# Jennifer03333333332/Soft-Rendering-Toolsets

Hardware: AMD Instinct MI355X
Metric: Mrays/s (higher is better)
Workload: dtype f32; 1 GPU; Scotty3D Pathtracer: Cornell box (cbox: area light + MIS, mirror + glass spheres), 1024x1024, 64 spp per step (52 steps = 3328 spp; 32 steps = BASELINE configs[3] 2048 spp), depth 8, BVH on; tiles=32x32 round-robin over ranks, collective=none (1 GPU), seed=0

## Files before the change

include/srt_pt_debug.h:

```cpp
#ifndef SRT_PT_DEBUG_H
#define SRT_PT_DEBUG_H

#include "srt_pt.h"

#ifdef __cplusplus
extern "C" {
#endif

int srt_pt_set_kernel(srt_pt* pt, int mode);
int srt_pt_section_cycles(srt_pt* pt, uint64_t out[8], int reset);

int srt_pt_kernel_time(srt_pt* pt, int enable, double* total_ms, uint64_t* launches);

int srt_pt_stream_times(srt_pt* pt, int enable, double ms_out[4], uint64_t* generations);
int srt_pt_stream_counters(srt_pt* pt, uint64_t out[4], int reset);
int srt_pt_kernel_form(srt_pt* pt, int* form);

int srt_pt_counters(srt_pt* pt, uint64_t out[8]);
int srt_pt_scene_counts(srt_pt* pt, uint64_t out[8]);
int srt_pt_refit_count(srt_pt* pt, uint64_t* refits);
int srt_pt_top_refit_count(srt_pt* pt, uint64_t* refits);
int srt_pt_top_refit_pending(srt_pt* pt, uint64_t out[2]);
int srt_pt_mesh_refit_pending(srt_pt* pt, uint64_t out[2]);
long srt_pt_dump_lights(srt_pt* pt, int from_device, uint32_t* heads, float* mats, size_t cap_lights, float* tris, size_t cap_tris);
int srt_pt_dump_shading(srt_pt* pt, int from_device, uint32_t counts[2], srt_pt_material* materials, size_t cap_materials, uint32_t* light_heads,
                        float* light_values, size_t cap_lights, uint32_t* env_type, float env_radiance[3]);
int srt_pt_math_cos_sin(srt_pt* pt, const float* x, size_t n, float* cos_out, float* sin_out);
int srt_pt_math_sincos2(srt_pt* pt, const float* x, size_t n, float* cos_out, float* sin_out);
int srt_pt_math_atan2(srt_pt* pt, const float* y, const float* x, size_t n, float* out);
int srt_pt_math_acos(srt_pt* pt, const float* x, size_t n, float* out);
int srt_pt_math_hypot(srt_pt* pt, const float* x, const float* y, size_t n, float* out);
int srt_pt_rig_posed_host(uint32_t njoints, const int32_t* parent, const float* extents, const float base[3], const float* rest_pose,
                          const uint32_t* knot_offsets, const float* knot_times, const float* knot_quats, float t, float* euler_out, float* posed_out);
int srt_pt_rig_step_ik_host(uint32_t njoints, const int32_t* parent, const float* extents, float* pose_inout, const uint32_t* handle_joints,
                            const float* targets, const uint8_t* enabled, uint32_t nhandles, uint32_t calls);
int srt_pt_emitter_advance_host(srt_pt_emitter* em, float dt, uint32_t* substeps, uint32_t* spawns_out, uint32_t cap, int* cleared, double schedule_out[2]);

int srt_pt_math_exp(srt_pt* pt, const float* x, size_t n, float* out);
int srt_pt_math_pow(srt_pt* pt, const float* x, const float* y, size_t n, float* out);
int srt_pt_math_div_sqrt(srt_pt* pt, const float* in, size_t lanes, int shared_c2, float* out);
int srt_pt_math_tri_verdict(srt_pt* pt, const float* in, size_t lanes, float* out);
int srt_pt_math_leaf_fold(srt_pt* pt, const float* in, size_t lanes, float* out);
int srt_pt_math_sphere_batch(srt_pt* pt, const float* in, size_t lanes, float* out);
int srt_pt_math_box_sweep(srt_pt* pt, const float* in, size_t lanes, float* out);
int srt_pt_math_point_affine(srt_pt* pt, const float* in, size_t lanes, float* out);

int srt_pt_live_resources(uint64_t out[3]);

#ifdef __cplusplus
}
#endif
#endif
```

soft-rendering-toolsets_amd/_pt_bindings.py:

```python
from __future__ import annotations

import ctypes
import os
import weakref
from ctypes import POINTER, c_float, c_int, c_long, c_size_t, c_uint32, c_uint64, c_void_p

import numpy as np


class PtMaterial(ctypes.Structure):
    _fields_ = [("type", c_uint32), ("a", c_float * 3), ("b", c_float * 3), ("ior", c_float)]


LOGGED_RAY_DTYPE = np.dtype([("point", np.float32, 3), ("dir", np.float32, 3), ("t", np.float32), ("pixel", np.uint32),
                             ("sample", np.uint32), ("bounce", np.uint32)])
SRT_CANCELLED = 1


class SrtCancelled(Exception):
    """A render call returned SRT_CANCELLED: srt_pt_cancel cut it short, its output was not written."""


_HIP_MEMCPY_D2H = 2

# ... 136 lines not shown
    lib.srt_pt_dump_bvh.restype = c_long
    lib.srt_pt_counters.argtypes = [c_void_p, c_void_p]
    lib.srt_pt_math_cos_sin.argtypes = [c_void_p, c_void_p, c_size_t, c_void_p, c_void_p]
    lib.srt_pt_math_sincos2.argtypes = [c_void_p, c_void_p, c_size_t, c_void_p, c_void_p]
    lib.srt_pt_math_acos.argtypes = [c_void_p, c_void_p, c_size_t, c_void_p]
    lib.srt_pt_math_atan2.argtypes = [c_void_p, c_void_p, c_void_p, c_size_t, c_void_p]
    lib.srt_pt_set_elision.argtypes = [c_void_p, c_int]
    lib.srt_pt_rays_elided.argtypes = [c_void_p, POINTER(c_uint64), c_int]
    lib.srt_pt_set_normal_colors.argtypes = [c_void_p, c_int]
    lib.srt_pt_group_set_normal_colors.argtypes = [c_void_p, c_int]
    lib.srt_pt_set_dynamic_lights.argtypes = [c_void_p, c_int]
    lib.srt_pt_group_set_dynamic_lights.argtypes = [c_void_p, c_int]
    lib.srt_pt_dump_lights.argtypes = [c_void_p, c_int, c_void_p, c_void_p, c_size_t, c_void_p, c_size_t]
    lib.srt_pt_dump_lights.restype = c_long
    lib.srt_pt_math_exp.argtypes = [c_void_p, c_void_p, c_size_t, c_void_p]
    lib.srt_pt_math_pow.argtypes = [c_void_p, c_void_p, c_void_p, c_size_t, c_void_p]
    lib.srt_pt_tonemap.argtypes = [c_void_p, c_void_p, c_uint32, c_uint32, c_float, c_void_p]
    lib.srt_pt_tonemap_device.argtypes = [c_void_p, c_void_p, c_void_p, c_uint32, c_uint32, c_float, c_void_p]
    lib.srt_pt_math_div_sqrt.argtypes = [c_void_p, c_void_p, c_size_t, ctypes.c_int, c_void_p]
    lib.srt_pt_math_tri_verdict.argtypes = [c_void_p, c_void_p, c_size_t, c_void_p]
    lib.srt_pt_math_leaf_fold.argtypes = [c_void_p, c_void_p, c_size_t, c_void_p]
    lib.srt_pt_math_box_sweep.argtypes = [c_void_p, c_void_p, c_size_t, c_void_p]
    lib.srt_pt_math_point_affine.argtypes = [c_void_p, c_void_p, c_size_t, c_void_p]
    lib.srt_pt_math_sphere_batch.argtypes = [c_void_p, c_void_p, c_size_t, c_void_p]
    lib.srt_pt_sync.argtypes = [c_void_p]
    lib.srt_pt_cancel.argtypes = [c_void_p]
    lib.srt_pt_cancel_requested.argtypes = [c_void_p]
    lib.srt_pt_clear_cancel.argtypes = [c_void_p]
    lib.srt_pt_set_ray_log.argtypes = [c_void_p, c_uint32]
    lib.srt_pt_read_ray_log.argtypes = [c_void_p, c_void_p, c_size_t, POINTER(c_size_t), POINTER(c_uint64)]
    lib.srt_pt_read_ray_log_stream.argtypes = [c_void_p, c_void_p, c_void_p, c_size_t, POINTER(c_size_t), POINTER(c_uint64)]
    lib.srt_pt_group_render_epoch_lane.argtypes = [c_void_p, c_int, c_uint64, c_uint32, c_uint32, POINTER(c_void_p), POINTER(c_void_p)]
    lib.srt_pt_group_cancel.argtypes = [c_void_p]
    lib.srt_pt_group_clear_cancel.argtypes = [c_void_p]
    lib.srt_pt_group_set_ray_log.argtypes = [c_void_p, c_uint32]
    lib.srt_pt_group_read_ray_log.argtypes = [c_void_p, c_int, c_void_p, c_size_t, POINTER(c_size_t), POINTER(c_uint64)]
    lib.srt_pt_max_samples_per_launch.argtypes = [c_void_p, POINTER(c_uint32)]
    lib.srt_pt_accumulator_floats.argtypes = [c_void_p, POINTER(c_size_t)]
    lib.srt_pt_render_samples_device.argtypes = [c_void_p, c_void_p, c_uint64, c_uint32, c_uint32]
    lib.srt_pt_fold_epochs_device.argtypes = [c_void_p, c_void_p, c_uint32, c_uint32, c_uint32, c_uint32, c_void_p]
    lib.srt_pt_accumulator_tiles_device.argtypes = [c_void_p, c_void_p, c_void_p, c_void_p]
    lib.srt_pt_group_reset_accumulator.argtypes = [c_void_p]
    lib.srt_pt_group_max_samples_per_launch.argtypes = [c_void_p, POINTER(c_uint32)]
    lib.srt_pt_group_render_samples.argtypes = [c_void_p, c_int, c_uint64, c_uint32, c_uint32]
    lib.srt_pt_group_wait_lane.argtypes = [c_void_p, c_int]
    lib.srt_pt_group_fold.argtypes = [c_void_p, c_int, c_uint32, c_uint32, c_uint32, c_uint32]
# ... 1158 lines not shown
        self._check(self._lib, self._lib.srt_pt_math_sphere_batch(self._ctx, _p(planes), n, _p(out)))
        form = lambda b: {"hit": out[b:b + 9:3].T != 0, "t": out[b + 1:b + 9:3].T.copy(), "dist": out[b + 2:b + 9:3].T.copy()}
        return form(0), form(9), out[18:21].T.copy(), out[21] != 0

    def math_box_sweep(self, box, org, inv, times):
        box, org, inv, times = _f32(box).reshape(-1, 6), _f32(org).reshape(-1, 3), _f32(inv).reshape(-1, 3), _f32(times).reshape(-1, 2)
        n = len(box)
        assert len(org) == n and len(inv) == n and len(times) == n and n > 0
        planes = np.ascontiguousarray(np.concatenate([box, org, inv, times], axis=1).T)
        out = np.zeros((6, n), np.float32)
        self._check(self._lib, self._lib.srt_pt_math_box_sweep(self._ctx, _p(planes), n, _p(out)))
        form = lambda b: {"hit": out[b] != 0, "tx": out[b + 1].copy(), "ty": out[b + 2].copy()}
        return form(0), form(3)

    def math_point_affine(self, mats, points):
        mats, points = _f32(mats).reshape(-1, 16), _f32(points).reshape(-1, 3)
        W, n = len(mats), len(points)
        assert n == 64 * W and W > 0
        buf = np.ascontiguousarray(np.concatenate([mats.ravel(), points.T.ravel()]), np.float32)
        out = np.zeros((7, n), np.float32)
        self._check(self._lib, self._lib.srt_pt_math_point_affine(self._ctx, _p(buf), n, _p(out)))
        return out[0:3].T.copy(), out[3:6].T.copy(), out[6].reshape(W, 64)[:, 0] != 0

    def math_cos_sin(self, x):
        x = _f32(x)
        c, s = np.zeros_like(x), np.zeros_like(x)
        self._check(self._lib, self._lib.srt_pt_math_cos_sin(self._ctx, _p(x), len(x), _p(c), _p(s)))
        return c, s

    def math_sincos2(self, x):
        x = _f32(x)
        c, s = np.zeros_like(x), np.zeros_like(x)
        self._check(self._lib, self._lib.srt_pt_math_sincos2(self._ctx, _p(x), len(x), _p(c), _p(s)))
        return c, s

    def sync(self) -> None:
        self._check(self._lib, self._lib.srt_pt_sync(self._ctx))


class PathtracerGroup:

    def __init__(self, devices):
        from . import SrtError, _check, load_library

        self._SrtError, self._check = SrtError, _check
        self._lib = load_library()
# ... 252 lines not shown
```

soft-rendering-toolsets_amd/csrc/pt_probe.hip:

```cpp
#include <hip/hip_runtime.h>

#include "pt_anim.h"
#include "pt_context.h"
#include "pt_device.h"
#include "srt_pt_debug.h"

#include "pt_trace.h"

namespace srt {

__global__ void pt_math_kernel(const float* __restrict__ x, size_t n, float* __restrict__ c, float* __restrict__ s) {
  const size_t i = (size_t)blockIdx.x * blockDim.x + threadIdx.x;
  if (i < n) { c[i] = srt_cosf(x[i]); s[i] = srt_sinf(x[i]); }
}

__global__ void pt_sincos2_kernel(const float* __restrict__ x, size_t n, float* __restrict__ c, float* __restrict__ s) {
  const size_t i = (size_t)blockIdx.x * blockDim.x + threadIdx.x;
  float cv, sv;
  srt_sincosf2(x[i < n ? i : n - 1], cv, sv);
  if (i < n) { c[i] = cv; s[i] = sv; }
}

__global__ void pt_acos_kernel(const float* __restrict__ x, size_t n, float* __restrict__ out) {
  const size_t i = (size_t)blockIdx.x * blockDim.x + threadIdx.x;
// ... 175 lines not shown
  const float bx[6] = {v[0], v[1], v[2], v[3], v[4], v[5]};
  const V3 org = v3(v[6], v[7], v[8]), inv = v3(v[9], v[10], v[11]);
  float ax = v[12], ay = v[13], bxx = v[12], bxy = v[13];
  const bool ha = box_hit_inv(bx, org, inv, ax, ay);
  const bool hb = box_hit_rec(bx, org, inv, bxx, bxy);
  out[i] = ha ? 1.0f : 0.0f; out[lanes + i] = ax; out[2 * lanes + i] = ay;
  out[3 * lanes + i] = hb ? 1.0f : 0.0f; out[4 * lanes + i] = bxx; out[5 * lanes + i] = bxy;
}

__global__ void pt_point_affine_kernel(const float* __restrict__ in, size_t lanes, float* __restrict__ out) {
  const size_t i = (size_t)blockIdx.x * blockDim.x + threadIdx.x;
  if (i >= lanes) return;
  Mat4 m;
#pragma unroll
  for (int j = 0; j < 16; j++) m.c[j / 4][j % 4] = in[(i / 64) * 16 + j];
  const float* pl = in + (lanes / 64) * 16;
  const V3 v = v3(pl[i], pl[lanes + i], pl[2 * lanes + i]);
  bool skipped = false;
  const V3 a = mat_point_affine(m, mat_affine_row(m), v, &skipped);
  const V3 b = mat_point(m, v);
  out[i] = a.x; out[lanes + i] = a.y; out[2 * lanes + i] = a.z;
  out[3 * lanes + i] = b.x; out[4 * lanes + i] = b.y; out[5 * lanes + i] = b.z;
  out[6 * lanes + i] = skipped ? 1.0f : 0.0f;
}

}

using namespace srt;

namespace {

template <size_t K, size_t M, class Launch>
int math_round_trip(srt_pt* pt, const char* what, const float* const (&in)[K], size_t in_floats, float* const (&out)[M], size_t out_floats, Launch&& launch) {
  int st = need_device(pt, what);
  if (st != SRT_OK) return st;
  for (const float* p : in) if (!p) return srt::fail(SRT_ERR_INVALID, "%s: NULL argument", what);
  for (const float* p : out) if (!p) return srt::fail(SRT_ERR_INVALID, "%s: NULL argument", what);
  if (!in_floats) return SRT_OK;
  DeviceBuffer<float> din_own[K], dout_own[M];
  float *din[K], *dout[M];
  for (size_t k = 0; k < K; k++) { if ((st = din_own[k].ensure(in_floats))) return st; din[k] = din_own[k]; }
  for (size_t m = 0; m < M; m++) { if ((st = dout_own[m].ensure(out_floats))) return st; dout[m] = dout_own[m]; }
  for (size_t k = 0; k < K; k++) SRT_HIP(hipMemcpyAsync(din[k], in[k], in_floats * 4, hipMemcpyHostToDevice, pt->stream));
  launch(din, dout);
  SRT_HIP(hipGetLastError());
  for (size_t m = 0; m < M; m++) SRT_HIP(hipMemcpyAsync(out[m], dout[m], out_floats * 4, hipMemcpyDeviceToHost, pt->stream));
// ... 73 lines not shown
      if (ntri < 1 || ntri > 12) return srt::fail(SRT_ERR_INVALID, "srt_pt_math_leaf_fold: wave %zu has %u triangles (1..12)", w, ntri);
    }
  const size_t in_floats = (lanes / 64) * kLeafFoldWave + 18 * lanes;
  return math_round_trip(pt, "srt_pt_math_leaf_fold", {in}, in_floats, {out}, 25 * lanes, [&](float* const* d, float* const* o) {
    pt_leaf_fold_kernel<<<math_grid(lanes), dim3(256), 0, pt->stream>>>(d[0], lanes, o[0]); });
}

int srt_pt_math_sphere_batch(srt_pt* pt, const float* in, size_t lanes, float* out) {
  return math_round_trip(pt, "srt_pt_math_sphere_batch", {in}, 19 * lanes, {out}, 22 * lanes, [&](float* const* d, float* const* o) {
    pt_sphere_batch_kernel<<<math_grid(lanes), dim3(256), 0, pt->stream>>>(d[0], lanes, o[0]); });
}

int srt_pt_math_box_sweep(srt_pt* pt, const float* in, size_t lanes, float* out) {
  return math_round_trip(pt, "srt_pt_math_box_sweep", {in}, 14 * lanes, {out}, 6 * lanes, [&](float* const* d, float* const* o) {
    pt_box_sweep_kernel<<<math_grid(lanes), dim3(256), 0, pt->stream>>>(d[0], lanes, o[0]); });
}

int srt_pt_math_point_affine(srt_pt* pt, const float* in, size_t lanes, float* out) {
  if (lanes % 64) return srt::fail(SRT_ERR_INVALID, "srt_pt_math_point_affine: %zu lanes are not whole waves of 64", lanes);
  return math_round_trip(pt, "srt_pt_math_point_affine", {in}, (lanes / 64) * 16 + 3 * lanes, {out}, 7 * lanes, [&](float* const* d, float* const* o) {
    pt_point_affine_kernel<<<math_grid(lanes), dim3(256), 0, pt->stream>>>(d[0], lanes, o[0]); });
}

}
```

soft-rendering-toolsets_amd/csrc/pt_trace.h:

```cpp
#ifndef SRT_PT_TRACE_H
#define SRT_PT_TRACE_H

#include "pt_device.h"
#include "pt_scene.h"

namespace srt {

constexpr int kMaxPathDepth = 16;

struct DScene {
  const Node* nodes;
  const Tri* tris;
  const TriNrm* tri_nrm;
  const Object* objects;
  const Light* lights;
  const LightTri* light_tris;
  const Material* materials;
  const WaveInterior* wave_tlas;
  const WaveInterior* blas_recs;
  const uint32_t* wave_lazy;
  const DeltaLight* delta_lights;
  uint32_t ndelta;
  uint32_t env_type;
  float env_radiance[3];
// ... 159 lines not shown
  const float lx = (b0 - o.x) * inv.x, hx = (b3 - o.x) * inv.x;
  const float ly = (b1 - o.y) * inv.y, hy = (b4 - o.y) * inv.y;
  const float lz = (b2 - o.z) * inv.z, hz = (b5 - o.z) * inv.z;
  float tmin = sx ? hx : lx;
  float tmax = sx ? lx : hx;
  const float tymin = sy ? hy : ly;
  const float tymax = sy ? ly : hy;
  const bool miss_y = (tmin > tymax) | (tymin > tmax);
  tmin = (tymin > tmin) ? tymin : tmin;
  tmax = (tymax < tmax) ? tymax : tmax;
  const float tzmin = sz ? hz : lz;
  const float tzmax = sz ? lz : hz;
  const bool miss_z = (tmin > tzmax) | (tzmin > tmax);
  tmin = (tzmin > tmin) ? tzmin : tmin;
  tmax = (tzmax < tmax) ? tzmax : tmax;
  const bool hit = !(miss_y | miss_z);
  const float nx = ((tmin >= tx) & (tmin <= ty)) ? tmin : tx;
  const float ny = ((tmax >= nx) & (tmax <= ty)) ? tmax : ty;
  tx = hit ? nx : tx;
  ty = hit ? ny : ty;
  return hit;
}

SRT_DEV uint32_t topdown_step(const WaveInterior& W, V3 org, V3 inv, float tx, float ty, float rb0, float rb1,
                              float& farx, float& lx, float& ly, float& rx, float& ry) {
  float t1x = tx, t1y = ty, t2x = tx, t2y = ty;
  const bool hl = box_hit_inv(W.boxl, org, inv, t1x, t1y);
  const bool hr = box_hit_inv(W.boxr, org, inv, t2x, t2y);
  const bool hb = hl & hr;
  const bool cl = (hb & (t1x < t2x)) | (!hb & hl);
  const bool own_l = hl, own_r = hr | !hl;
  farx = hb ? (cl ? t2x : t1x) : rb0;
  lx = own_l ? t1x : rb0; ly = own_l ? t1y : rb1;
  rx = own_r ? t2x : rb0; ry = own_r ? t2y : rb1;
  return (hl ? 1u : 0u) | (hr ? 2u : 0u) | (cl ? 4u : 0u) | (hb ? 8u : 0u);
}

struct RecFrame { int32_t second; float a, b; uint32_t flags; };
template <int MAXD, bool COUNT>
SRT_DEV Hit traverse_records(const DScene& S, const Object& o, const Ray& ray, float tx, float ty, Counters& cnt) {
  const WaveInterior* __restrict__ recs = S.blas_recs + o.rec_base;
  const V3 inv = v3(1.0f / ray.d.x, 1.0f / ray.d.y, 1.0f / ray.d.z);
  RecFrame stack[MAXD];
  int sp = 0;
  int32_t cur = 0;
  Hit ret;
  for (;;) {
    if (COUNT) cnt.v[C_BLAS]++;
    ret.hit = false; ret.dist = 0.0f; ret.obj = 0; ret.tri = 0;
    bool descended = false;
    if (cur < 0) {
// ... 563 lines not shown
```

soft-rendering-toolsets_amd/csrc/pt_wave.h:

```cpp
#ifndef SRT_PT_WAVE_H
#define SRT_PT_WAVE_H


#include "pt_trace.h"
#include "pt_flat.h"
#include "pt_stream.h"

namespace srt {

constexpr uint32_t kWaveMaxObjects = 16;
constexpr uint32_t kChunk = 64;
constexpr uint32_t kBurst = 3;
constexpr uint32_t kMissTri = 0xFFFFFFFFu;
constexpr uint32_t kFlatReady = 16;
constexpr int kRecFields = 8;

struct WaveParams {
  TileMap T;
  uint64_t seed;
  uint32_t sample_base;
  uint32_t samples;
  uint32_t groups3, singles;
  uint32_t units3;
  uint32_t total_units;
  uint32_t nlanes;
// ... 286 lines not shown
    }
  }
}

enum { ST_REFILL = 0, ST_TOPDOWN, ST_LEAVES, ST_COMBINE, ST_POST, ST_SHADE, ST_TERMINATE, ST_COUNT_ };
template <bool IN_LDS> struct ColdU32;
template <> struct ColdU32<false> {
  uint32_t v;
  SRT_DEV void bind(uint32_t*) {}
  SRT_DEV operator uint32_t() const { return v; }
  SRT_DEV ColdU32& operator=(uint32_t x) { v = x; return *this; }
  SRT_DEV ColdU32& operator=(const ColdU32& o) { v = o.v; return *this; }
};
template <> struct ColdU32<true> {
  uint32_t* p;
  SRT_DEV void bind(uint32_t* at) { p = at; }
  SRT_DEV operator uint32_t() const { return *p; }
  SRT_DEV ColdU32& operator=(uint32_t x) { *p = x; return *this; }
  SRT_DEV ColdU32& operator=(const ColdU32& o) { *p = *o.p; return *this; }
};
constexpr int kColdWords = 4;
__host__ __device__ constexpr bool cold_in_lds(int trav) { return trav == 0; }

template <bool STAMP, int TRAV, bool DL, int NR, int PHASE = 0>
#ifndef SRT_WAVE_OCC
#define SRT_WAVE_OCC 4
#endif
#ifndef SRT_WAVE_OCC2
#define SRT_WAVE_OCC2 5
#endif
#ifndef SRT_WAVE_OCC2T
#define SRT_WAVE_OCC2T 4
#endif
#ifndef SRT_WAVE_OCC3T
#define SRT_WAVE_OCC3T 4
#endif
#ifndef SRT_STREAM_OCC
#define SRT_STREAM_OCC 4
#endif
#ifndef SRT_PROBE_OCC
#define SRT_PROBE_OCC 8
#endif
__global__ __launch_bounds__(256, PHASE == 2 ? SRT_PROBE_OCC : TRAV == 4 ? SRT_STREAM_OCC : (NR == 2 ? (TRAV == 1 ? SRT_WAVE_OCC2T : (TRAV >= 3 ? 4 : SRT_WAVE_OCC2)) : (TRAV == 1 ? SRT_WAVE_OCC3T : SRT_WAVE_OCC))) void pt_wave_kernel(DScene S_in, WaveParams P_in, const Object* __restrict__ a_objects,
                                                      const Tri* __restrict__ a_tris, const TriNrm* __restrict__ a_nrm,
                                                      const Node* __restrict__ a_nodes, const Light* __restrict__ a_lights,
                                                      const LightTri* __restrict__ a_ltris, const Material* __restrict__ a_mats,
                                                      const WaveInterior* __restrict__ a_wave, const WaveInterior* __restrict__ a_blas,
                                                      float* __restrict__ a_records, float* __restrict__ a_samples) {
  static_assert(NR == 3 || (NR == 2 && TRAV != 2 && !DL), "two-ray batches: sweep builds without delta / environment lights only");
  static_assert(!(STAMP && TRAV >= 3), "the streamed builds have no section stamps");
  static_assert(PHASE == 0 || (TRAV == 4 && !DL), "split generations: the streamed sweeps without delta / environment lights");
  constexpr int C = NR - 1;
  constexpr bool STREAM = TRAV >= 3;
  constexpr bool LAZY = TRAV == 1 || TRAV == 4;
  constexpr bool LEAF_ONCE = !(STAMP && TRAV == 1) && !(TRAV == 4 && DL && PHASE == 0);
  if constexpr (STREAM) {
    if (P_in.sc->done != 0u) return;
  }
  if (cancel_raised(P_in.dev_cancel)) return;
  if constexpr (!STREAM) {
    if (P_in.watch != 0u && blockIdx.x == gridDim.x - 1u) {
      if (threadIdx.x != 0u) return;
      for (;;) {
        if (cancel_requested(P_in.host_cancel)) {
          atomicExch(P_in.dev_cancel, 1u);
          atomicMax(P_in.queue_head, kQueuePoison);
          return;
        }
        if (__hip_atomic_load(P_in.queue_head, __ATOMIC_RELAXED, __HIP_MEMORY_SCOPE_AGENT) >= (unsigned long long)P_in.total_units) return;
        __builtin_amdgcn_s_sleep(127);
        __builtin_amdgcn_s_sleep(127);
      }
    }
  }
  DScene S = S_in;
  S.objects = a_objects; S.tris = a_tris; S.tri_nrm = a_nrm; S.nodes = a_nodes; S.lights = a_lights;
  S.light_tris = a_ltris; S.materials = a_mats; S.wave_tlas = a_wave; S.blas_recs = a_blas;
  WaveParams P = P_in;
// ... 54 lines not shown
  Rng rng;
  rng.state = 0; rng.inc = 1; rng.draws = 0;
  V3 org = v3(0, 0, 0);
  V3 d[NR];
#pragma unroll
  for (int j = 0; j < NR; j++) d[j] = v3(0.25f, 0.5f, 0.75f);
  float cb0 = 0.0f, cb1 = 0.0f;
  bool actA = false, actB = false;
  Spec att = spec(0, 0, 0);
  float pdf4 = 1.0f, pdf_area = 0.0f;
  bool discrete = false;

  bool sh_phase = false, sa1 = false, sa2 = false;
  uint32_t light_i = 0, held_chit = kRetMiss;
  Spec pl = spec(0, 0, 0), dA_keep = spec(0, 0, 0), d6_keep = spec(0, 0, 0);
  V3 dC_keep = v3(0, 0, 1);
  float sb1[3] = {0.0f, 0.0f, 0.0f};

  FlatState FS;
  FlatFrame fstack[TRAV == 2 ? kFlatStack : 1];
  bool need_begin = false;

  uint32_t chunk_next = 0, chunk_end = 0;
  bool queue_empty = false;
  uint32_t units_finished = 0;

#define ST(w) __builtin_nontemporal_load(P.state + ((size_t)(w) * P.nlanes + lane_global))
#define ST_SET(w, v) __builtin_nontemporal_store((uint32_t)(v), P.state + ((size_t)(w) * P.nlanes + lane_global))
#define REC_AT(lev, half) (reinterpret_cast<f32x4*>(P.records) + (((size_t)lane_global * kMaxPathDepth + (size_t)(lev)) * 2u + (half)))
#define REC_STORE(lev, half, x, y, z, w) __builtin_nontemporal_store(f32x4{x, y, z, w}, REC_AT(lev, half))
#define REC_LOAD(lev, half) (*REC_AT(lev, half))
  uint32_t emit_mask = 0;
  if constexpr (STREAM && PHASE == 2) {
    const uint32_t fw = has_slot ? ST(SW_FLAGS) : 0u;
    alive = (fw & 1u) != 0;
    if (alive) {
      burst = (fw & 2u) != 0; actA = (fw & 4u) != 0; actB = (fw & 8u) != 0;
      org = v3(__uint_as_float(ST(SW_ORG)), __uint_as_float(ST(SW_ORG + 1)), __uint_as_float(ST(SW_ORG + 2)));
      d[C] = v3(__uint_as_float(ST(SW_DC)), __uint_as_float(ST(SW_DC + 1)), __uint_as_float(ST(SW_DC + 2)));
      cb0 = __uint_as_float(ST(SW_CB0)); cb1 = __uint_as_float(ST(SW_CB1));
      d[0] = v3(__uint_as_float(ST(SW_D0)), __uint_as_float(ST(SW_D0 + 1)), __uint_as_float(ST(SW_D0 + 2)));
      if (NR > 2) d[1] = v3(__uint_as_float(ST(SW_D1)), __uint_as_float(ST(SW_D1 + 1)), __uint_as_float(ST(SW_D1 + 2)));
    }
  } else if constexpr (STREAM) {
    if (P.gen == 0u && lane_phys == 0u) { P.sc->nrays[1] = 0u; P.sc->cast_head[1] = 0u; P.sc->alive[1] = 0u; P.sc->alive_n[1] = 0u; }
    const uint32_t fw = has_slot ? ST(SW_FLAGS) : 0u;
    alive = (fw & 1u) != 0;
// ... 54 lines not shown
      ST_SET(SW_PEND0, pend0);
      if (NR > 2) ST_SET(SW_PEND1, pend1);
      ST_SET(SW_RNG_LO, (uint32_t)rng.state); ST_SET(SW_RNG_HI, (uint32_t)(rng.state >> 32));
      ST_SET(SW_ORG, __float_as_uint(org.x)); ST_SET(SW_ORG + 1, __float_as_uint(org.y)); ST_SET(SW_ORG + 2, __float_as_uint(org.z));
      ST_SET(SW_DC, __float_as_uint(d[C].x)); ST_SET(SW_DC + 1, __float_as_uint(d[C].y)); ST_SET(SW_DC + 2, __float_as_uint(d[C].z));
      ST_SET(SW_CB0, __float_as_uint(cb0)); ST_SET(SW_CB1, __float_as_uint(cb1));
      ST_SET(SW_ATT, __float_as_uint(att.r)); ST_SET(SW_ATT + 1, __float_as_uint(att.g)); ST_SET(SW_ATT + 2, __float_as_uint(att.b));
      ST_SET(SW_PDF4, __float_as_uint(pdf4)); ST_SET(SW_PDF_AREA, __float_as_uint(pdf_area));
      if constexpr (DL || TRAV == 4) {
        ST_SET(SW_D0, __float_as_uint(d[0].x)); ST_SET(SW_D0 + 1, __float_as_uint(d[0].y)); ST_SET(SW_D0 + 2, __float_as_uint(d[0].z));
        if (NR > 2) { ST_SET(SW_D1, __float_as_uint(d[1].x)); ST_SET(SW_D1 + 1, __float_as_uint(d[1].y)); ST_SET(SW_D1 + 2, __float_as_uint(d[1].z)); }
      }
      if constexpr (DL) {
        ST_SET(SW_LIGHT_I, light_i); ST_SET(SW_HELD, held_chit);
        ST_SET(SW_PL, __float_as_uint(pl.r)); ST_SET(SW_PL + 1, __float_as_uint(pl.g)); ST_SET(SW_PL + 2, __float_as_uint(pl.b));
        ST_SET(SW_DA, __float_as_uint(dA_keep.r)); ST_SET(SW_DA + 1, __float_as_uint(dA_keep.g)); ST_SET(SW_DA + 2, __float_as_uint(dA_keep.b));
        ST_SET(SW_D6, __float_as_uint(d6_keep.r)); ST_SET(SW_D6 + 1, __float_as_uint(d6_keep.g)); ST_SET(SW_D6 + 2, __float_as_uint(d6_keep.b));
        ST_SET(SW_DCK, __float_as_uint(dC_keep.x)); ST_SET(SW_DCK + 1, __float_as_uint(dC_keep.y)); ST_SET(SW_DCK + 2, __float_as_uint(dC_keep.z));
        ST_SET(SW_SB1, __float_as_uint(sb1[0])); ST_SET(SW_SB1 + 1, __float_as_uint(sb1[1])); ST_SET(SW_SB1 + 2, __float_as_uint(sb1[2]));
      }
    }
  };

  for (int pass = (PHASE == 2 ? 1 : 0);; pass++) {
    const unsigned long long need = (!STREAM || (PHASE != 1 && pass == 1)) ? __ballot(!alive && has_slot) : 0ull;
    uint32_t stream_unit = kMissTri;
    if constexpr (STREAM && PHASE != 1) {
      if (pass == 1) {
        const uint32_t want = (uint32_t)__popcll(need);
        const uint32_t my_rank = __builtin_amdgcn_mbcnt_hi((uint32_t)(need >> 32), __builtin_amdgcn_mbcnt_lo((uint32_t)need, 0u));
        if (lane == 0) s_blk[wave] = want;
        __syncthreads();
        if (threadIdx.x == 0) {
          unsigned long long total = 0;
          for (uint32_t w = 0; w < blockDim.x / 64u; w++) { const unsigned long long n_ = s_blk[w]; s_blk[w] = total; total += n_; }
          s_blk[32] = total ? atomicAdd(P.queue_head, total) : (unsigned long long)P.total_units;
        }
        __syncthreads();
        const unsigned long long u = s_blk[32] + s_blk[wave] + my_rank;
        if (!alive && has_slot && u < (unsigned long long)P.total_units) stream_unit = (uint32_t)u;
        __syncthreads();
      }
    }
    if ((!STREAM && need != 0ull && !(queue_empty && chunk_next == chunk_end)) || (STREAM && PHASE != 1 && pass == 1)) {
      const uint32_t want = (uint32_t)__popcll(need);
      const uint32_t my_rank = __builtin_amdgcn_mbcnt_hi((uint32_t)(need >> 32), __builtin_amdgcn_mbcnt_lo((uint32_t)need, 0u));
      uint32_t given = 0, my_unit = stream_unit;
      while (!STREAM && given < want) {
        if (chunk_next == chunk_end) {
          if (queue_empty) break;
          unsigned long long start = 0;
          const uint32_t grab = P.chunk;
          if (lane == 0) {
            start = atomicAdd(P.queue_head, (unsigned long long)grab);
          }
          start = __shfl(start, 0);
          if (start >= P.total_units) { queue_empty = true; break; }
          chunk_next = (uint32_t)start;
          chunk_end = (uint32_t)(start + grab < P.total_units ? start + grab : P.total_units);
        }
        const uint32_t avail = chunk_end - chunk_next;
        const uint32_t take = avail < want - given ? avail : want - given;
        if (!alive && my_rank >= given && my_rank < given + take) my_unit = chunk_next + (my_rank - given);
        chunk_next += take;
        given += take;
      }
      if (my_unit != kMissTri) {
        uint32_t x, y;
        const uint32_t g3 = opq(P.groups3), g1 = opq(P.singles), n3 = opq(P.units3), img_w = opq(S.w), img_h = opq(S.h);
        uint32_t u_pixel, u_first, u_count;
        if (my_unit < n3) { u_pixel = my_unit / g3; u_first = (my_unit % g3) * (uint32_t)NR; u_count = (uint32_t)NR; }
        else { const uint32_t v = my_unit - n3; u_pixel = v / g1; u_first = g3 * (uint32_t)NR + v % g1; u_count = 1u; }
        unit_pixel(opq(P.T), u_pixel, x, y);
        if (x < img_w && y < img_h) {
          alive = true;
          burst = true;
          pxy = x | (y << 16);
          pixel_slot = u_pixel;
          samp = u_first | (u_first << 16) | (u_count << 30);
          level = 0;
// ... 28 lines not shown
#pragma unroll
        for (int r = 0; r < NR; r++) { eact[r] = alive; eb1[r] = cb1; }
        if (DL && sh_phase) {
          if (NR > 1) eact[1] = alive && sa1;
          if (NR > 2) eact[NR - 1] = alive && sa2;
#pragma unroll
          for (int r = 0; r < NR; r++) eb1[r] = sb1[r];
        } else if (burst) { if (NR > 1) eact[1] = alive && actA; if (NR > 2) eact[NR - 1] = alive && actB; }
        else if (NR == 3) { eact[0] = alive && actA; eact[1] = alive && actB; }
#pragma unroll
        for (int r = 0; r < NR; r++) {
          if (eact[r]) {
            const size_t i = (size_t)r * P.nlanes + lane_global;
            nt_store_ray(P.ray_o, 2 * i, org.x, org.y, org.z, cb0);
            nt_store_ray(P.ray_d, 2 * i, d[r].x, d[r].y, d[r].z, eb1[r]);
            emit_mask |= 1u << r;
          }
        }
        save_state();
        break;
      }
    } else {
      if (__ballot(alive) == 0ull) {
        if (queue_empty && chunk_next == chunk_end) break;
        continue;
      }
    }
    SECTION_END(ST_REFILL)

    if constexpr (TRAV == 4 && PHASE == 2) {
      bool pact[NR];
#pragma unroll
      for (int r = 0; r < NR; r++) pact[r] = alive;
      if (burst) { if (NR > 1) pact[1] = alive && actA; if (NR > 2) pact[NR - 1] = alive && actB; }
      else if (NR == 3) { pact[0] = alive && actA; pact[1] = alive && actB; }
      float pb0[NR], pb1[NR];
#pragma unroll
      for (int r = 0; r < NR; r++) { pb0[r] = cb0; pb1[r] = cb1; }
      auto is_lazy = [&](uint32_t k) { const Object& ob = S.objects[k]; return ob.kind == OBJ_MESH && ob.use_bvh != 0u && ob.nrec > 0u; };
      bool h_[NR]; float dd_[NR]; uint32_t tt_[NR];
      if (Q == 0) {
        for (uint32_t k = 0; k < nobj; k++)
          if (is_lazy(k)) object_queueN<NR>(S, k, org, d, pb0, pb1, h_, dd_, tt_, pact, P, lane_global, true, emit_mask);
      } else {
        V3 pinv[NR];
#pragma unroll
        for (int r = 0; r < NR; r++) pinv[r] = v3(1.0f / d[r].x, 1.0f / d[r].y, 1.0f / d[r].z);
// ... 55 lines not shown
        cnt.v[C_RAYS] += 1u + (actA ? 1u : 0u) + (actB ? 1u : 0u);
        flat_begin(FS, S, org, d[0], d[1], d[2], cb0, cb1, burst || actA, burst ? actA : actB, burst ? actB : true);
        need_begin = false;
      }
      flat_run(FS, fstack, S, org, d[0], d[1], d[2], cb0, cb1, alive, P.flat_ready, P.flat_interior);
      batch_ready = alive && FS.mode == FM_DONE;
      res[0] = FS.res0; res[1] = FS.res1; res[2] = FS.res2;
      SECTION_END(ST_LEAVES)
    } else if (Q == 0) {
      PHit acc[NR];
#pragma unroll
      for (int r = 0; r < NR; r++) acc[r] = packed_miss();
      for (uint32_t k = 0; k < nobj; k++) {
        bool h[NR]; float dd[NR]; uint32_t tt[NR];
        object_testN<LAZY, NR, TRAV == 4, LEAF_ONCE>(S, k, org, d, rb0, rb1, cnt, h, dd, tt, act, cidx, &P, lane_global, pass == 1, &emit_mask);
#pragma unroll
        for (int r = 0; r < NR; r++) packed_fold(acc[r], h[r], dd[r], (k << 27) | tt[r]);
      }
#pragma unroll
      for (int r = 0; r < NR; r++) res[r] = unpack_ret(acc[r].dist, acc[r].id);
    } else {
      V3 inv[NR];
      float tx0[NR], ty0[NR];
      unsigned long long fl[NR];
      float farx0[NR];
#pragma unroll
      for (int r = 0; r < NR; r++) {
        fl[r] = 0ull; farx0[r] = 0.0f;
        inv[r] = v3(1.0f / d[r].x, 1.0f / d[r].y, 1.0f / d[r].z);
        const float dn = norm(d[r]);
        tx0[r] = rb0[r] / dn; ty0[r] = rb1[r] / dn;
      }
      auto topdown = [&]() {
        for (uint32_t q = 0; q < Q; q++) {
          const WaveInterior& W = S.wave_tlas[q];
#pragma unroll
          for (int r = 0; r < NR; r++) {
            float tx = tx0[r], ty = ty0[r];
            if (q != 0) { tx = SLOT(q, r, 0); ty = SLOT(q, r, 1); }
            float fx, lx, ly, rx, ry;
            const uint32_t f = topdown_step(W, org, inv[r], tx, ty, rb0[r], rb1[r], fx, lx, ly, rx, ry);
            fl[r] |= (unsigned long long)f << (4 * q);
            if (q != 0) SLOT(q, r, 0) = fx; else farx0[r] = fx;
            if (W.l_ref >= 0) { SLOT(W.l_ref, r, 0) = lx; SLOT(W.l_ref, r, 1) = ly; }
            if (W.r_ref >= 0) { SLOT(W.r_ref, r, 0) = rx; SLOT(W.r_ref, r, 1) = ry; }
          }
        }
      };
      topdown();
      SECTION_END(ST_TOPDOWN)
      for (int q = (int)Q - 1; q >= 0; q--) {
        const WaveInterior& W = S.wave_tlas[q];
        PHit L[NR], R[NR];
        auto lazy_leaf = [&](int32_t ref, uint32_t n) {
          if (!LAZY || ref >= 0 || n != 1u) return false;
          const Object& ob = S.objects[(uint32_t)~ref];
          return ob.kind == OBJ_MESH && ob.use_bvh != 0u && ob.nrec > 0u;
        };
        auto eval_child = [&](int32_t ref, uint32_t n, PHit* out, const bool* need) {
          if (ref >= 0) {
#pragma unroll
            for (int r = 0; r < NR; r++) { out[r].dist = SLOT(ref, r, 0); out[r].id = __float_as_uint(SLOT(ref, r, 1)); }
          } else {
#pragma unroll
            for (int r = 0; r < NR; r++) out[r] = packed_miss();
            const uint32_t first = (uint32_t)~ref;
            for (uint32_t k = first; k < first + n; k++) {
              bool h[NR]; float dd[NR]; uint32_t tt[NR];
              object_testN<TRAV == 1, NR, false, LEAF_ONCE>(S, k, org, d, rb0, rb1, cnt, h, dd, tt, need, cidx);
#pragma unroll
              for (int r = 0; r < NR; r++) packed_fold(out[r], h[r], dd[r], (k << 27) | tt[r]);
            }
          }
        };
        auto need_of = [&](bool is_left, const PHit* other, bool other_known, bool* need) {
#pragma unroll
          for (int r = 0; r < NR; r++) {
            const uint32_t f = (uint32_t)(fl[r] >> (4 * q)) & 15u;
            const bool nearer = ((f & 4u) != 0) == is_left;
            const float farx = (q != 0) ? SLOT(q, r, 0) : farx0[r];
            const bool second = !other_known | (farx < other[r].dist) | ((other[r].id == kRetMiss) & ((f & 8u) != 0));
            need[r] = act[r] & ((f & 3u) != 0) & (nearer | second);
          }
        };
        if constexpr (!LAZY) {
          eval_child(W.l_ref, W.l_cnt, L, act);
          eval_child(W.r_ref, W.r_cnt, R, act);
        } else if constexpr (TRAV == 4) {
          const uint32_t lz = S.wave_lazy[q];
          const bool lazy_l = lazy_leaf(W.l_ref, W.l_cnt), lazy_r = lazy_leaf(W.r_ref, W.r_cnt);
          auto queued = [&](int32_t ref, bool is_left, const PHit* other, bool other_known, PHit* out) {
            bool need[NR], h[NR]; float dd[NR]; uint32_t tt[NR];
            need_of(is_left, other, other_known, need);
            const uint32_t k = (uint32_t)~ref;
            object_queueN<NR>(S, k, org, d, rb0, rb1, h, dd, tt, need, P, lane_global, pass == 1, emit_mask);
#pragma unroll
            for (int r = 0; r < NR; r++) { out[r] = packed_miss(); packed_fold(out[r], h[r], dd[r], (k << 27) | tt[r]); }
          };
#pragma unroll
          for (int r = 0; r < NR; r++) { L[r] = packed_miss(); R[r] = packed_miss(); }
          if (pass == 1) {
// ... 15 lines not shown
#pragma nounroll
        for (int t = 0; t < 2; t++) {
          const bool left = (t == 0) != right_first;
          const int32_t ref = left ? W.l_ref : W.r_ref;
          const uint32_t n = left ? W.l_cnt : W.r_cnt;
          bool need[NR];
          if (left ? lazy_l : lazy_r) need_of(left, first_out, t == 1 && !(TRAV == 4 && (lz & (left ? 2u : 1u)) != 0u), need);
          else {
#pragma unroll
            for (int r = 0; r < NR; r++) need[r] = act[r];
          }
          PHit out[NR];
          eval_child(ref, n, out, need);
#pragma unroll
          for (int r = 0; r < NR; r++) {
            if (t == 0) first_out[r] = out[r];
            if (left) L[r] = out[r]; else R[r] = out[r];
          }
        }
        }
        SECTION_END(ST_LEAVES)
#pragma unroll
        for (int r = 0; r < NR; r++) {
          const uint32_t f = (uint32_t)(fl[r] >> (4 * q)) & 15u;
          const float farx = (q != 0) ? SLOT(q, r, 0) : farx0[r];
          const PHit ret = packed_combine(L[r], R[r], (f & 3u) != 0, (f & 4u) != 0, (f & 8u) != 0, farx);
          if (q > 0) { SLOT(q, r, 0) = ret.dist; SLOT(q, r, 1) = __uint_as_float(ret.id); }
          else res[r] = unpack_ret(ret.dist, ret.id);
        }
        SECTION_END(ST_COMBINE)
      }
    }

    if constexpr (TRAV == 4) {
      if (pass == 1) {
        save_state();
        break;
      }
    }
    if (batch_ready) {
      uint32_t chit = kRetMiss;
      bool more_shadow = false;
      bool shadow_returned = false;
      if constexpr (DL) {
        if (sh_phase) {
          shadow_returned = true;
#pragma unroll
// ... 320 lines not shown
```

Baseline: 10950 Mrays/s.

## Add min/max slab box test fast path and store per-node flags in LDS slots

Adds a branch-free min/max slab test for top-down TLAS traversal. It is used when a wave-wide check shows all boxes, ray origins and inverse directions are finite and nonzero, so the NaN/inf handling of the general box test can be skipped. The 64-bit packed per-node flag word is replaced by storing each node's flags in the existing LDS slot (fl0 for the root), which lowers register pressure but adds LDS reads in the bottom-up pass. A probe kernel and binding are added to test the fast path, and it is only active when SRT_EXACT_FAST_PATHS is set and for TRAV==0 without DL.

```diff
diff --git a/include/srt_pt_debug.h b/include/srt_pt_debug.h
--- a/include/srt_pt_debug.h
+++ b/include/srt_pt_debug.h
@@ -44,6 +44,7 @@
 int srt_pt_math_sphere_batch(srt_pt* pt, const float* in, size_t lanes, float* out);
 int srt_pt_math_box_sweep(srt_pt* pt, const float* in, size_t lanes, float* out);
 int srt_pt_math_point_affine(srt_pt* pt, const float* in, size_t lanes, float* out);
+int srt_pt_math_topdown_minmax(srt_pt* pt, const float* in, size_t lanes, float* out);
 
 int srt_pt_live_resources(uint64_t out[3]);
 
diff --git a/soft-rendering-toolsets_amd/_pt_bindings.py b/soft-rendering-toolsets_amd/_pt_bindings.py
--- a/soft-rendering-toolsets_amd/_pt_bindings.py
+++ b/soft-rendering-toolsets_amd/_pt_bindings.py
@@ -182,6 +182,7 @@
     lib.srt_pt_math_leaf_fold.argtypes = [c_void_p, c_void_p, c_size_t, c_void_p]
     lib.srt_pt_math_box_sweep.argtypes = [c_void_p, c_void_p, c_size_t, c_void_p]
     lib.srt_pt_math_point_affine.argtypes = [c_void_p, c_void_p, c_size_t, c_void_p]
+    lib.srt_pt_math_topdown_minmax.argtypes = [c_void_p, c_void_p, c_size_t, c_void_p]
     lib.srt_pt_math_sphere_batch.argtypes = [c_void_p, c_void_p, c_size_t, c_void_p]
     lib.srt_pt_sync.argtypes = [c_void_p]
     lib.srt_pt_cancel.argtypes = [c_void_p]
@@ -1386,6 +1387,20 @@
         self._check(self._lib, self._lib.srt_pt_math_point_affine(self._ctx, _p(buf), n, _p(out)))
         return out[0:3].T.copy(), out[3:6].T.copy(), out[6].reshape(W, 64)[:, 0] != 0
 
+    def math_topdown_minmax(self, records, rays):
+        records = np.ascontiguousarray(records, np.uint32).reshape(-1, 7, 16)
+        rays = _f32(rays).reshape(-1, 10)
+        W, n = len(records), len(rays)
+        assert n == 64 * W and W > 0
+        buf = np.ascontiguousarray(np.concatenate([records.ravel().view(np.float32), rays.T.ravel()]), np.float32)
+        out = np.zeros((85, n), np.float32)
+        self._check(self._lib, self._lib.srt_pt_math_topdown_minmax(self._ctx, _p(buf), n, _p(out)))
+        bits = out[:84].view(np.uint32)
+        form = lambda b: np.ascontiguousarray(bits[b:b + 42].reshape(7, 6, n).transpose(2, 0, 1))
+        took = out[84].reshape(W, 64) != 0
+        assert (took == took[:, :1]).all()
+        return form(0), form(42), took[:, 0]
+
     def math_cos_sin(self, x):
         x = _f32(x)
         c, s = np.zeros_like(x), np.zeros_like(x)
diff --git a/soft-rendering-toolsets_amd/csrc/pt_probe.hip b/soft-rendering-toolsets_amd/csrc/pt_probe.hip
--- a/soft-rendering-toolsets_amd/csrc/pt_probe.hip
+++ b/soft-rendering-toolsets_amd/csrc/pt_probe.hip
@@ -1,4 +1,6 @@
 #include <hip/hip_runtime.h>
+
+#include <type_traits>
 
 #include "pt_anim.h"
 #include "pt_context.h"
@@ -221,6 +223,50 @@
   out[i] = a.x; out[lanes + i] = a.y; out[2 * lanes + i] = a.z;
   out[3 * lanes + i] = b.x; out[4 * lanes + i] = b.y; out[5 * lanes + i] = b.z;
   out[6 * lanes + i] = skipped ? 1.0f : 0.0f;
+}
+
+constexpr int kProbeQ = 7;
+__global__ void pt_topdown_minmax_kernel(const float* __restrict__ in, size_t lanes, float* __restrict__ out) {
+  __shared__ float s_slot[4][kProbeQ][2][64];
+  const size_t i = (size_t)blockIdx.x * blockDim.x + threadIdx.x;
+  if (i >= lanes) return;
+  const int lane = threadIdx.x & 63, wave = threadIdx.x >> 6;
+  const size_t w = (size_t)(uint32_t)__builtin_amdgcn_readfirstlane((int)(i / 64));
+  const WaveInterior* __restrict__ recs = reinterpret_cast<const WaveInterior*>(in) + w * kProbeQ;
+  const float* pl = in + (lanes / 64) * kProbeQ * 16;
+  float v[10];
+#pragma unroll
+  for (int j = 0; j < 10; j++) v[j] = pl[(size_t)j * lanes + i];
+  const V3 org = v3(v[0], v[1], v[2]), inv = v3(v[3], v[4], v[5]);
+  const float tx0 = v[6], ty0 = v[7], rb0 = v[8], rb1 = v[9];
+#define PSLOT(q, f) s_slot[wave][q][f][lane]
+  bool bok = true;
+  if (lane < kProbeQ) {
+    const bool l = minmax_box_ok(recs[lane].boxl), r = minmax_box_ok(recs[lane].boxr);
+    bok = l & r;
+  }
+  const bool boxes_ok = __ballot(!bok) == 0ull;
+  const bool org_ok = minmax_origin_ok(org), inv_ok = minmax_inv_ok(inv);
+  const bool ok = org_ok & inv_ok;
+  const bool fast = boxes_ok && __ballot(!ok) == 0ull;
+  auto sweep = [&](auto minmax, float* __restrict__ o) {
+    for (int q = 0; q < kProbeQ; q++) {
+      const WaveInterior& W = recs[q];
+      float tx = tx0, ty = ty0;
+      if (q != 0) { tx = PSLOT(q, 0); ty = PSLOT(q, 1); }
+      float fx, lx, ly, rx, ry;
+      const uint32_t f = topdown_step<decltype(minmax)::value>(W, org, inv, tx, ty, rb0, rb1, fx, lx, ly, rx, ry);
+      if (q != 0) { PSLOT(q, 0) = fx; PSLOT(q, 1) = __uint_as_float(f); }
+      if (W.l_ref >= 0) { PSLOT(W.l_ref, 0) = lx; PSLOT(W.l_ref, 1) = ly; }
+      if (W.r_ref >= 0) { PSLOT(W.r_ref, 0) = rx; PSLOT(W.r_ref, 1) = ry; }
+      float* p = o + (size_t)(6 * q) * lanes + i;
+      p[0] = __uint_as_float(f); p[lanes] = fx; p[2 * lanes] = lx; p[3 * lanes] = ly; p[4 * lanes] = rx; p[5 * lanes] = ry;
+    }
+  };
+  if (fast) sweep(std::true_type{}, out); else sweep(std::false_type{}, out);
+  sweep(std::false_type{}, out + (size_t)(6 * kProbeQ) * lanes);
+  out[(size_t)(12 * kProbeQ) * lanes + i] = fast ? 1.0f : 0.0f;
+#undef PSLOT
 }
 
 }
@@ -340,4 +386,20 @@
     pt_point_affine_kernel<<<math_grid(lanes), dim3(256), 0, pt->stream>>>(d[0], lanes, o[0]); });
 }
 
-}
+int srt_pt_math_topdown_minmax(srt_pt* pt, const float* in, size_t lanes, float* out) {
+  if (lanes % 64) return srt::fail(SRT_ERR_INVALID, "srt_pt_math_topdown_minmax: %zu lanes are not whole waves of 64", lanes);
+  if (in)
+    for (size_t w = 0; w < lanes / 64; w++)
+      for (int q = 0; q < kProbeQ; q++) {
+        WaveInterior W;
+        __builtin_memcpy(&W, in + (w * kProbeQ + (size_t)q) * 16, sizeof(W));
+        for (int32_t ref : {W.l_ref, W.r_ref})
+          if (ref >= 0 && (ref <= q || ref >= kProbeQ))
+            return srt::fail(SRT_ERR_INVALID, "srt_pt_math_topdown_minmax: wave %zu, node %d has child %d (a leaf, or %d..%d)", w, q, ref, q + 1, kProbeQ - 1);
+      }
+  const size_t in_floats = (lanes / 64) * kProbeQ * 16 + 10 * lanes;
+  return math_round_trip(pt, "srt_pt_math_topdown_minmax", {in}, in_floats, {out}, (12 * kProbeQ + 1) * lanes, [&](float* const* d, float* const* o) {
+    pt_topdown_minmax_kernel<<<math_grid(lanes), dim3(256), 0, pt->stream>>>(d[0], lanes, o[0]); });
+}
+
+}
diff --git a/soft-rendering-toolsets_amd/csrc/pt_trace.h b/soft-rendering-toolsets_amd/csrc/pt_trace.h
--- a/soft-rendering-toolsets_amd/csrc/pt_trace.h
+++ b/soft-rendering-toolsets_amd/csrc/pt_trace.h
@@ -205,11 +205,53 @@
   return hit;
 }
 
+SRT_DEV bool class_finite_nonzero(float v) {
+#if defined(__HIP_DEVICE_COMPILE__)
+  return __builtin_amdgcn_classf(v, 0x198);
+#else
+  return finite_f(v) && v != 0.0f;
+#endif
+}
+SRT_DEV bool minmax_origin_ok(V3 o) {
+  const bool x = class_finite(o.x), y = class_finite(o.y), z = class_finite(o.z);
+  return x & y & z;
+}
+SRT_DEV bool minmax_inv_ok(V3 inv) {
+  const bool x = class_finite_nonzero(inv.x), y = class_finite_nonzero(inv.y), z = class_finite_nonzero(inv.z);
+  return x & y & z;
+}
+SRT_DEV bool minmax_box_ok(const float* __restrict__ bx) {
+  bool ok = true;
+#pragma unroll
+  for (int a = 0; a < 3; a++) {
+    const bool lo = finite_f(bx[a]), hi = finite_f(bx[3 + a]);
+    ok = ok & lo & hi & (bx[a] <= bx[3 + a]);
+  }
+  return ok;
+}
+
+SRT_DEV bool box_hit_minmax(const float* __restrict__ bx, V3 o, V3 inv, float& tx, float& ty) {
+  const float b0 = bx[0], b1 = bx[1], b2 = bx[2], b3 = bx[3], b4 = bx[4], b5 = bx[5];
+  const float lx = (b0 - o.x) * inv.x, hx = (b3 - o.x) * inv.x;
+  float tmin = __builtin_fminf(lx, hx), tmax = __builtin_fmaxf(lx, hx);
+  const float ly = (b1 - o.y) * inv.y, hy = (b4 - o.y) * inv.y;
+  tmin = __builtin_fmaxf(tmin, __builtin_fminf(ly, hy)); tmax = __builtin_fminf(tmax, __builtin_fmaxf(ly, hy));
+  const float lz = (b2 - o.z) * inv.z, hz = (b5 - o.z) * inv.z;
+  tmin = __builtin_fmaxf(tmin, __builtin_fminf(lz, hz)); tmax = __builtin_fminf(tmax, __builtin_fmaxf(lz, hz));
+  const bool hit = !(tmin > tmax);
+  const bool in1 = hit & (tmin >= tx) & (tmin <= ty);
+  const bool in2 = hit & (in1 | (tmax >= tx)) & (tmax <= ty);
+  tx = in1 ? tmin : tx;
+  ty = in2 ? tmax : ty;
+  return hit;
+}
+
+template <bool MINMAX = false>
 SRT_DEV uint32_t topdown_step(const WaveInterior& W, V3 org, V3 inv, float tx, float ty, float rb0, float rb1,
                               float& farx, float& lx, float& ly, float& rx, float& ry) {
   float t1x = tx, t1y = ty, t2x = tx, t2y = ty;
-  const bool hl = box_hit_inv(W.boxl, org, inv, t1x, t1y);
-  const bool hr = box_hit_inv(W.boxr, org, inv, t2x, t2y);
+  const bool hl = MINMAX ? box_hit_minmax(W.boxl, org, inv, t1x, t1y) : box_hit_inv(W.boxl, org, inv, t1x, t1y);
+  const bool hr = MINMAX ? box_hit_minmax(W.boxr, org, inv, t2x, t2y) : box_hit_inv(W.boxr, org, inv, t2x, t2y);
   const bool hb = hl & hr;
   const bool cl = (hb & (t1x < t2x)) | (!hb & hl);
   const bool own_l = hl, own_r = hr | !hl;
diff --git a/soft-rendering-toolsets_amd/csrc/pt_wave.h b/soft-rendering-toolsets_amd/csrc/pt_wave.h
--- a/soft-rendering-toolsets_amd/csrc/pt_wave.h
+++ b/soft-rendering-toolsets_amd/csrc/pt_wave.h
@@ -1,6 +1,8 @@
 #ifndef SRT_PT_WAVE_H
 #define SRT_PT_WAVE_H
 
+
+#include <type_traits>
 
 #include "pt_trace.h"
 #include "pt_flat.h"
@@ -333,6 +335,22 @@
 constexpr int kColdWords = 4;
 __host__ __device__ constexpr bool cold_in_lds(int trav) { return trav == 0; }
 
+template <bool WITH_BOXES> struct WaveFlags;
+template <> struct WaveFlags<false> {
+  bool empty_ = false;
+  SRT_DEV bool queue_empty() const { return empty_; }
+  SRT_DEV void set_queue_empty() { empty_ = true; }
+  SRT_DEV bool boxes_ok() const { return false; }
+  SRT_DEV void set_boxes_ok() {}
+};
+template <> struct WaveFlags<true> {
+  uint32_t bits_ = 0u;
+  SRT_DEV bool queue_empty() const { return (bits_ & 1u) != 0u; }
+  SRT_DEV void set_queue_empty() { bits_ |= 1u; }
+  SRT_DEV bool boxes_ok() const { return (bits_ & 2u) != 0u; }
+  SRT_DEV void set_boxes_ok() { bits_ |= 2u; }
+};
+
 template <bool STAMP, int TRAV, bool DL, int NR, int PHASE = 0>
 #ifndef SRT_WAVE_OCC
 #define SRT_WAVE_OCC 4
@@ -365,6 +383,7 @@
   constexpr bool STREAM = TRAV >= 3;
   constexpr bool LAZY = TRAV == 1 || TRAV == 4;
   constexpr bool LEAF_ONCE = !(STAMP && TRAV == 1) && !(TRAV == 4 && DL && PHASE == 0);
+  constexpr bool MINMAX = SRT_EXACT_FAST_PATHS && TRAV == 0 && !DL && PHASE == 0;
   if constexpr (STREAM) {
     if (P_in.sc->done != 0u) return;
   }
@@ -465,7 +484,7 @@
   bool need_begin = false;
 
   uint32_t chunk_next = 0, chunk_end = 0;
-  bool queue_empty = false;
+  WaveFlags<MINMAX> wflags;
   uint32_t units_finished = 0;
 
 #define ST(w) __builtin_nontemporal_load(P.state + ((size_t)(w) * P.nlanes + lane_global))
@@ -566,6 +585,16 @@
     }
   };
 
+  if constexpr (MINMAX) {
+    bool ok = true;
+    for (uint32_t q = (uint32_t)lane; q < Q; q += 64u) {
+      const WaveInterior& W = S.wave_tlas[q];
+      const bool l = minmax_box_ok(W.boxl), r = minmax_box_ok(W.boxr);
+      ok = ok & l & r;
+    }
+    if (__ballot(!ok) == 0ull) wflags.set_boxes_ok();
+  }
+
   for (int pass = (PHASE == 2 ? 1 : 0);; pass++) {
     const unsigned long long need = (!STREAM || (PHASE != 1 && pass == 1)) ? __ballot(!alive && has_slot) : 0ull;
     uint32_t stream_unit = kMissTri;
@@ -586,20 +615,20 @@
         __syncthreads();
       }
     }
-    if ((!STREAM && need != 0ull && !(queue_empty && chunk_next == chunk_end)) || (STREAM && PHASE != 1 && pass == 1)) {
+    if ((!STREAM && need != 0ull && !(wflags.queue_empty() && chunk_next == chunk_end)) || (STREAM && PHASE != 1 && pass == 1)) {
       const uint32_t want = (uint32_t)__popcll(need);
       const uint32_t my_rank = __builtin_amdgcn_mbcnt_hi((uint32_t)(need >> 32), __builtin_amdgcn_mbcnt_lo((uint32_t)need, 0u));
       uint32_t given = 0, my_unit = stream_unit;
       while (!STREAM && given < want) {
         if (chunk_next == chunk_end) {
-          if (queue_empty) break;
+          if (wflags.queue_empty()) break;
           unsigned long long start = 0;
           const uint32_t grab = P.chunk;
           if (lane == 0) {
             start = atomicAdd(P.queue_head, (unsigned long long)grab);
           }
           start = __shfl(start, 0);
-          if (start >= P.total_units) { queue_empty = true; break; }
+          if (start >= P.total_units) { wflags.set_queue_empty(); break; }
           chunk_next = (uint32_t)start;
           chunk_end = (uint32_t)(start + grab < P.total_units ? start + grab : P.total_units);
         }
@@ -674,7 +703,7 @@
       }
     } else {
       if (__ballot(alive) == 0ull) {
-        if (queue_empty && chunk_next == chunk_end) break;
+        if (wflags.queue_empty() && chunk_next == chunk_end) break;
         continue;
       }
     }
@@ -776,16 +805,16 @@
     } else {
       V3 inv[NR];
       float tx0[NR], ty0[NR];
-      unsigned long long fl[NR];
+      uint32_t fl0[NR];
       float farx0[NR];
 #pragma unroll
       for (int r = 0; r < NR; r++) {
-        fl[r] = 0ull; farx0[r] = 0.0f;
+        fl0[r] = 0u; farx0[r] = 0.0f;
         inv[r] = v3(1.0f / d[r].x, 1.0f / d[r].y, 1.0f / d[r].z);
         const float dn = norm(d[r]);
         tx0[r] = rb0[r] / dn; ty0[r] = rb1[r] / dn;
       }
-      auto topdown = [&]() {
+      auto topdown = [&](auto minmax) {
         for (uint32_t q = 0; q < Q; q++) {
           const WaveInterior& W = S.wave_tlas[q];
 #pragma unroll
@@ -793,15 +822,21 @@
             float tx = tx0[r], ty = ty0[r];
             if (q != 0) { tx = SLOT(q, r, 0); ty = SLOT(q, r, 1); }
             float fx, lx, ly, rx, ry;
-            const uint32_t f = topdown_step(W, org, inv[r], tx, ty, rb0[r], rb1[r], fx, lx, ly, rx, ry);
-            fl[r] |= (unsigned long long)f << (4 * q);
-            if (q != 0) SLOT(q, r, 0) = fx; else farx0[r] = fx;
+            const uint32_t f = topdown_step<decltype(minmax)::value>(W, org, inv[r], tx, ty, rb0[r], rb1[r], fx, lx, ly, rx, ry);
+            if (q != 0) { SLOT(q, r, 0) = fx; SLOT(q, r, 1) = __uint_as_float(f); } else { farx0[r] = fx; fl0[r] = f; }
             if (W.l_ref >= 0) { SLOT(W.l_ref, r, 0) = lx; SLOT(W.l_ref, r, 1) = ly; }
             if (W.r_ref >= 0) { SLOT(W.r_ref, r, 0) = rx; SLOT(W.r_ref, r, 1) = ry; }
           }
         }
       };
-      topdown();
+      bool batch_ok = false;
+      if constexpr (MINMAX) {
+        bool ok = minmax_origin_ok(org);
+#pragma unroll
+        for (int r = 0; r < NR; r++) { const bool inv_ok = minmax_inv_ok(inv[r]); ok = ok & inv_ok; }
+        batch_ok = wflags.boxes_ok() && __ballot(!ok) == 0ull;
+      }
+      if (MINMAX && batch_ok) topdown(std::true_type{}); else topdown(std::false_type{});
       SECTION_END(ST_TOPDOWN)
       for (int q = (int)Q - 1; q >= 0; q--) {
         const WaveInterior& W = S.wave_tlas[q];
@@ -830,7 +865,7 @@
         auto need_of = [&](bool is_left, const PHit* other, bool other_known, bool* need) {
 #pragma unroll
           for (int r = 0; r < NR; r++) {
-            const uint32_t f = (uint32_t)(fl[r] >> (4 * q)) & 15u;
+            const uint32_t f = (q != 0) ? __float_as_uint(SLOT(q, r, 1)) : fl0[r];
             const bool nearer = ((f & 4u) != 0) == is_left;
             const float farx = (q != 0) ? SLOT(q, r, 0) : farx0[r];
             const bool second = !other_known | (farx < other[r].dist) | ((other[r].id == kRetMiss) & ((f & 8u) != 0));
@@ -892,7 +927,7 @@
         SECTION_END(ST_LEAVES)
 #pragma unroll
         for (int r = 0; r < NR; r++) {
-          const uint32_t f = (uint32_t)(fl[r] >> (4 * q)) & 15u;
+          const uint32_t f = (q != 0) ? __float_as_uint(SLOT(q, r, 1)) : fl0[r];
           const float farx = (q != 0) ? SLOT(q, r, 0) : farx0[r];
           const PHit ret = packed_combine(L[r], R[r], (f & 3u) != 0, (f & 4u) != 0, (f & 8u) != 0, farx);
           if (q > 0) { SLOT(q, r, 0) = ret.dist; SLOT(q, r, 1) = __uint_as_float(ret.id); }
```

New measurement: 11300 Mrays/s (median of 6 runs). 3.1% higher.
